# xxlong0/NeuralUDF

Hardware: NVIDIA H100
Metric: ray-samples/sec (render_core fwd+bwd) (higher is better)
Workload: dtype f32

## Files before the change

### neuraludf_b200/csrc/gemm_tc.cuh

```cuda
#pragma once
#include <cuda.h>
#include <cudaTypedefs.h>
#include <cuda_bf16.h>

#include "gemm_simt.cuh"

namespace nudf {
namespace tc {

constexpr int BM = 128;
constexpr int BN = 128;
constexpr int BK = 64;
constexpr int THREADS = 256;
constexpr int A_HALF_BYTES = BM * BK * 2;
constexpr int B_HALF_BYTES = BN * BK * 2;
__host__ __device__ constexpr int b_plane_bytes(int wn) { return wn * BK * 2; }
__host__ __device__ constexpr int acc_ld(int wn) { return wn + 4; }

__host__ __device__ inline int pad16(int n) { return (n + 15) & ~15; }
__host__ __device__ inline int pad64(int k) { return (k + 63) & ~63; }

__host__ __device__ inline uint32_t sw128(uint32_t row, uint32_t k) {
  return (row >> 3) * 1024u + (row & 7u) * 128u + ((((k >> 3) ^ (row & 7u)) & 7u) << 4) + ((k & 7u) << 1);
}

constexpr int TN_PS = 32;
constexpr int TN_RING = 4;
constexpr uint32_t TN_F32_OPND = TN_PS * BM * 4;
constexpr uint32_t TN_F32_STAGE = 2 * TN_F32_OPND;
constexpr uint32_t TN_PLANE = BM * TN_PS * 2;
constexpr uint32_t TN_PLANE_STAGE = 4 * TN_PLANE;
struct TnMaps { CUtensorMap a, b; };
__host__ __device__ inline uint32_t sw128_mn(uint32_t mn, uint32_t k) {
  return (mn >> 6) * 4096u + (k >> 3) * 1024u + (k & 7u) * 128u + ((((mn >> 3) ^ k) & 7u) << 4) + ((mn & 7u) << 1);
}

__device__ __forceinline__ uint32_t pack_bf16(float a, float b) {
  __nv_bfloat162 v = __floats2bfloat162_rn(a, b);
  return *reinterpret_cast<uint32_t*>(&v);
}
template <int NP>
__device__ __forceinline__ void split4(const float x[4], uint2 planes[NP]) {
  float r[4] = {x[0], x[1], x[2], x[3]};
#pragma unroll
  for (int p = 0; p < NP; ++p) {
    float h[4];
#pragma unroll
    for (int j = 0; j < 4; ++j) {
      h[j] = __bfloat162float(__float2bfloat16_rn(r[j]));
      r[j] -= h[j];
    }
    planes[p] = make_uint2(pack_bf16(h[0], h[1]), pack_bf16(h[2], h[3]));
  }
}
__host__ __device__ inline int nt_of(int np) { return np == 2 ? 256 : 128; }
__host__ __device__ inline int n_tiles(int N, int np) { return (N + nt_of(np) - 1) / nt_of(np); }
__host__ __device__ inline int tile_rows(int N, int t, int np) { int r = N - nt_of(np) * t; return pad16(r < nt_of(np) ? r : nt_of(np)); }
__host__ __device__ inline int64_t tile_elems(int N, int K, int t, int np) { return (int64_t)(pad64(K) / 64) * np * tile_rows(N, t, np) * 64; }
__host__ __device__ inline int64_t tile_offset(int N, int K, int t, int np) {
  int64_t o = 0;
  for (int i = 0; i < t; ++i) o += tile_elems(N, K, i, np);
  return o;
}
__host__ __device__ inline int64_t image_elems(int N, int K, int np) { return tile_offset(N, K, n_tiles(N, np), np); }

static __device__ __forceinline__ void tc_prep_weights_body(const float* __restrict__ W, int64_t ldw, int N, int K, int transposed, int np,
                                                            uint16_t* __restrict__ img, int64_t start, int64_t stride) {
  const int Kp = pad64(K);
  const int nt = n_tiles(N, np);
  int64_t total = 0;
  for (int t = 0; t < nt; ++t) total += (int64_t)tile_rows(N, t, np) * Kp;
  for (int64_t idx = start; idx < total; idx += stride) {
    int64_t rem = idx;
    int t = 0;
    while (rem >= (int64_t)tile_rows(N, t, np) * Kp) { rem -= (int64_t)tile_rows(N, t, np) * Kp; ++t; }
    const int rows = tile_rows(N, t, np);
    const int nl = (int)(rem / Kp), k = (int)(rem - (int64_t)nl * Kp);
    const int n = t * nt_of(np) + nl;
    float x = 0.f;
    if (n < N && k < K) x = transposed ? W[(int64_t)k * ldw + n] : W[(int64_t)n * ldw + k];
    const int s = k >> 6, kl = k & 63;
    uint16_t* base = img + tile_offset(N, K, t, np) + (int64_t)s * np * rows * 64;
    const uint32_t off = sw128((uint32_t)nl, (uint32_t)kl) >> 1;
    float r = x;
    for (int p = 0; p < np; ++p) {
      __nv_bfloat16 h = __float2bfloat16_rn(r);
      base[(int64_t)p * rows * 64 + off] = __bfloat16_as_ushort(h);
      r -= __bfloat162float(h);
    }
  }
}
static __global__ void tc_prep_weights_kernel(const float* __restrict__ W, int64_t ldw, int N, int K, int transposed, int np,
                                              uint16_t* __restrict__ img) {
  tc_prep_weights_body(W, ldw, N, K, transposed, np, img, (int64_t)blockIdx.x * blockDim.x + threadIdx.x, (int64_t)gridDim.x * blockDim.x);
}


__device__ __forceinline__ uint32_t smem_u32(const void* p) { return (uint32_t)__cvta_generic_to_shared(p); }
__device__ __forceinline__ uint8_t* align1024(uint8_t* p) {
  return reinterpret_cast<uint8_t*>((reinterpret_cast<uintptr_t>(p) + 1023) & ~(uintptr_t)1023);
}

__device__ __forceinline__ void mbar_init(uint64_t* bar, uint32_t count) {
  asm volatile("mbarrier.init.shared::cta.b64 [%0], %1;" ::"r"(smem_u32(bar)), "r"(count) : "memory");
}
__device__ __forceinline__ void mbar_arrive_expect_tx(uint64_t* bar, uint32_t bytes) {
  asm volatile("mbarrier.arrive.expect_tx.shared::cta.b64 _, [%0], %1;" ::"r"(smem_u32(bar)), "r"(bytes) : "memory");
}
__device__ __forceinline__ uint32_t mbar_try_wait(uint32_t addr, uint32_t parity) {
  uint32_t ok;
  asm volatile(
      "{\n"
      ".reg .pred p;\n"
      "mbarrier.try_wait.parity.shared::cta.b64 p, [%1], %2;\n"
      "selp.u32 %0, 1, 0, p;\n"
      "}\n"
      : "=r"(ok)
      : "r"(addr), "r"(parity)
// ... 74 lines not shown
        "=f"(d[37]), "=f"(d[38]), "=f"(d[39]), "=f"(d[40]), "=f"(d[41]), "=f"(d[42]), "=f"(d[43]), "=f"(d[44]), "=f"(d[45]),
        "=f"(d[46]), "=f"(d[47]), "=f"(d[48]), "=f"(d[49]), "=f"(d[50]), "=f"(d[51]), "=f"(d[52]), "=f"(d[53]), "=f"(d[54]),
        "=f"(d[55]), "=f"(d[56]), "=f"(d[57]), "=f"(d[58]), "=f"(d[59]), "=f"(d[60]), "=f"(d[61]), "=f"(d[62]), "=f"(d[63])
      : "l"(da), "l"(db), "r"(0u));
}

__device__ __forceinline__ void wgmma_256(float (&d)[128], uint64_t da, uint64_t db, uint32_t accumulate) {
  asm volatile(
      "{\n"
      ".reg .pred p;\n"
      "setp.ne.b32 p, %130, 0;\n"
      "wgmma.mma_async.sync.aligned.m64n256k16.f32.bf16.bf16 "
      "{%0, %1, %2, %3, %4, %5, %6, %7, %8, %9, %10, %11, %12, %13, %14, %15, %16, %17, %18, %19, %20, %21, %22, %23, %24, "
      "%25, %26, %27, %28, %29, %30, %31, %32, %33, %34, %35, %36, %37, %38, %39, %40, %41, %42, %43, %44, %45, %46, %47, "
      "%48, %49, %50, %51, %52, %53, %54, %55, %56, %57, %58, %59, %60, %61, %62, %63, %64, %65, %66, %67, %68, %69, %70, "
      "%71, %72, %73, %74, %75, %76, %77, %78, %79, %80, %81, %82, %83, %84, %85, %86, %87, %88, %89, %90, %91, %92, %93, "
      "%94, %95, %96, %97, %98, %99, %100, %101, %102, %103, %104, %105, %106, %107, %108, %109, %110, %111, %112, %113, "
      "%114, %115, %116, %117, %118, %119, %120, %121, %122, %123, %124, %125, %126, %127}, %128, %129, p, 1, 1, 0, 0;\n"
      "}\n"
      : "+f"(d[0]), "+f"(d[1]), "+f"(d[2]), "+f"(d[3]), "+f"(d[4]), "+f"(d[5]), "+f"(d[6]), "+f"(d[7]), "+f"(d[8]),
        "+f"(d[9]), "+f"(d[10]), "+f"(d[11]), "+f"(d[12]), "+f"(d[13]), "+f"(d[14]), "+f"(d[15]), "+f"(d[16]), "+f"(d[17]),
        "+f"(d[18]), "+f"(d[19]), "+f"(d[20]), "+f"(d[21]), "+f"(d[22]), "+f"(d[23]), "+f"(d[24]), "+f"(d[25]), "+f"(d[26]),
        "+f"(d[27]), "+f"(d[28]), "+f"(d[29]), "+f"(d[30]), "+f"(d[31]), "+f"(d[32]), "+f"(d[33]), "+f"(d[34]), "+f"(d[35]),
        "+f"(d[36]), "+f"(d[37]), "+f"(d[38]), "+f"(d[39]), "+f"(d[40]), "+f"(d[41]), "+f"(d[42]), "+f"(d[43]), "+f"(d[44]),
        "+f"(d[45]), "+f"(d[46]), "+f"(d[47]), "+f"(d[48]), "+f"(d[49]), "+f"(d[50]), "+f"(d[51]), "+f"(d[52]), "+f"(d[53]),
        "+f"(d[54]), "+f"(d[55]), "+f"(d[56]), "+f"(d[57]), "+f"(d[58]), "+f"(d[59]), "+f"(d[60]), "+f"(d[61]), "+f"(d[62]),
        "+f"(d[63]), "+f"(d[64]), "+f"(d[65]), "+f"(d[66]), "+f"(d[67]), "+f"(d[68]), "+f"(d[69]), "+f"(d[70]), "+f"(d[71]),
        "+f"(d[72]), "+f"(d[73]), "+f"(d[74]), "+f"(d[75]), "+f"(d[76]), "+f"(d[77]), "+f"(d[78]), "+f"(d[79]), "+f"(d[80]),
        "+f"(d[81]), "+f"(d[82]), "+f"(d[83]), "+f"(d[84]), "+f"(d[85]), "+f"(d[86]), "+f"(d[87]), "+f"(d[88]), "+f"(d[89]),
        "+f"(d[90]), "+f"(d[91]), "+f"(d[92]), "+f"(d[93]), "+f"(d[94]), "+f"(d[95]), "+f"(d[96]), "+f"(d[97]), "+f"(d[98]),
        "+f"(d[99]), "+f"(d[100]), "+f"(d[101]), "+f"(d[102]), "+f"(d[103]), "+f"(d[104]), "+f"(d[105]), "+f"(d[106]),
        "+f"(d[107]), "+f"(d[108]), "+f"(d[109]), "+f"(d[110]), "+f"(d[111]), "+f"(d[112]), "+f"(d[113]), "+f"(d[114]),
        "+f"(d[115]), "+f"(d[116]), "+f"(d[117]), "+f"(d[118]), "+f"(d[119]), "+f"(d[120]), "+f"(d[121]), "+f"(d[122]),
        "+f"(d[123]), "+f"(d[124]), "+f"(d[125]), "+f"(d[126]), "+f"(d[127])
      : "l"(da), "l"(db), "r"(accumulate));
}

template <int WN>
__device__ __forceinline__ void wgmma_n(float (&d)[WN / 2], uint64_t da, uint64_t db, uint32_t accumulate) {
  if constexpr (WN == 256) wgmma_256(d, da, db, accumulate);
  else wgmma_128(d, da, db, accumulate);
}
template <int NP, int WN>
__device__ __forceinline__ void mma_slice(float (&d)[WN / 2], uint32_t a, uint32_t a_stride, uint32_t b, uint32_t b_stride, bool zero_first) {
  auto desc = [](uint32_t base, uint32_t stride, int p, int j) { return make_desc(base + p * stride + 32u * j); };
#pragma unroll
  for (int j = 0; j < BK / 16; ++j) {
    const uint32_t acc0 = (zero_first && j == 0) ? 0u : 1u;
    if constexpr (NP == 2) {
      wgmma_n<WN>(d, desc(a, a_stride, 1, j), desc(b, b_stride, 0, j), acc0);
      wgmma_n<WN>(d, desc(a, a_stride, 0, j), desc(b, b_stride, 1, j), 1u);
      wgmma_n<WN>(d, desc(a, a_stride, 0, j), desc(b, b_stride, 0, j), 1u);
    } else {
      wgmma_n<WN>(d, desc(a, a_stride, 2, j), desc(b, b_stride, 0, j), acc0);
      wgmma_n<WN>(d, desc(a, a_stride, 0, j), desc(b, b_stride, 2, j), 1u);
      wgmma_n<WN>(d, desc(a, a_stride, 1, j), desc(b, b_stride, 1, j), 1u);
      wgmma_n<WN>(d, desc(a, a_stride, 1, j), desc(b, b_stride, 0, j), 1u);
      wgmma_n<WN>(d, desc(a, a_stride, 0, j), desc(b, b_stride, 1, j), 1u);
    }
  }
}
__device__ __forceinline__ void mma_slice_mn(float (&d)[64], uint32_t a, uint32_t b, bool zero_first) {
#pragma unroll
  for (int j = 0; j < TN_PS / 16; ++j) {
    const uint32_t acc0 = (zero_first && j == 0) ? 0u : 1u;
    const uint32_t aj = a + 2048u * j, bj = b + 2048u * j;
    wgmma_128<1>(d, make_desc_mn(aj + TN_PLANE), make_desc_mn(bj), acc0);
    wgmma_128<1>(d, make_desc_mn(aj), make_desc_mn(bj + TN_PLANE), 1u);
    wgmma_128<1>(d, make_desc_mn(aj), make_desc_mn(bj), 1u);
  }
}

template <int WN>
__device__ __forceinline__ void acc_to_smem(const float (&d)[WN / 2], float* acc_s, int wg, int wtid) {
  constexpr int LD = acc_ld(WN);
  const int r = 64 * wg + 16 * (wtid >> 5) + ((wtid & 31) >> 2);
  const int c = 2 * (wtid & 3);
#pragma unroll
  for (int g = 0; g < WN / 8; ++g) {
    *reinterpret_cast<float2*>(acc_s + r * LD + 8 * g + c) = make_float2(d[4 * g], d[4 * g + 1]);
    *reinterpret_cast<float2*>(acc_s + (r + 8) * LD + 8 * g + c) = make_float2(d[4 * g + 2], d[4 * g + 3]);
  }
}
template <int WN, class Epi>
__device__ __forceinline__ void tile_epilogue(const float* acc_s, int64_t m0, int64_t M, int n0, int n_valid_end, const Epi& epi, int tid) {
  constexpr int LD = acc_ld(WN);
  const int cq = tid & 31;
#pragma unroll 1
  for (int h = 0; h < WN / 128; ++h) {
    const int cl = 128 * h + 4 * cq;
    const int col = n0 + cl;
    int nv = n_valid_end - col;
    nv = nv < 4 ? nv : 4;
    if (nv <= 0) break;
    for (int r0 = tid >> 5; r0 < BM; r0 += 2 * (THREADS / 32)) {
      typename Epi::Aux aux[2];
#pragma unroll
      for (int i = 0; i < 2; ++i) {
        const int64_t row = m0 + r0 + i * (THREADS / 32);
        if (row < M) epi.load(row, col, nv, aux[i]);
      }
#pragma unroll
      for (int i = 0; i < 2; ++i) {
        const int r = r0 + i * (THREADS / 32);
        const int64_t row = m0 + r;
        if (row < M) {
          const float4 t = *reinterpret_cast<const float4*>(acc_s + r * LD + cl);
          const float x[4] = {t.x, t.y, t.z, t.w};
          epi.apply(row, col, x, nv, aux[i]);
        }
      }
    }
  }
}

template <int NT>
__device__ __forceinline__ void fetch_a(const float* __restrict__ A, int64_t lda, int64_t m0, int64_t M, int k0, int K, int tid,
                                        bool vec_ok, float4 (&v)[BM * 16 / NT]) {
  const int c = tid & 15;
  const int rsub = tid >> 4;
  const int k = k0 + c * 4;
#pragma unroll
  for (int pass = 0; pass < BM * 16 / NT; ++pass) {
    const int64_t row = m0 + pass * (NT / 16) + rsub;
    v[pass] = make_float4(0.f, 0.f, 0.f, 0.f);
    if (row < M) {
      const float* p = A + row * lda + k;
      if (vec_ok && k + 3 < K) {
        v[pass] = *reinterpret_cast<const float4*>(p);
      } else {
        if (k + 0 < K) v[pass].x = p[0];
        if (k + 1 < K) v[pass].y = p[1];
        if (k + 2 < K) v[pass].z = p[2];
        if (k + 3 < K) v[pass].w = p[3];
      }
    }
  }
}
template <int NP, int NT>
__device__ __forceinline__ void store_a(const float4 (&v)[BM * 16 / NT], uint8_t* sa, int tid) {
  const int c = tid & 15;
  const int rsub = tid >> 4;
#pragma unroll
  for (int pass = 0; pass < BM * 16 / NT; ++pass) {
    const float x[4] = {v[pass].x, v[pass].y, v[pass].z, v[pass].w};
    uint2 pl[NP];
    split4<NP>(x, pl);
    const uint32_t off = sw128((uint32_t)(pass * (NT / 16) + rsub), (uint32_t)(c * 4));
#pragma unroll
    for (int p = 0; p < NP; ++p) *reinterpret_cast<uint2*>(sa + p * A_HALF_BYTES + off) = pl[p];
  }
}
template <int NP, int NT>
__device__ __forceinline__ void stage_a_direct(const float* __restrict__ A, int64_t lda, int64_t m0, int64_t M, int k0, int K,
                                               uint8_t* sa, int tid, bool vec_ok) {
  float4 v[BM * 16 / NT];
  fetch_a<NT>(A, lda, m0, M, k0, K, tid, vec_ok, v);
  store_a<NP, NT>(v, sa, tid);
}

__device__ __forceinline__ void fetch_block_t(const float* __restrict__ X, int64_t ld, int m0, int m_total, int r0, int rows,
                                              int64_t k0, int64_t k_end, int lane, bool vec_ok, float4 (&v)[8][2]) {
  const int mq = lane & 7, kq = lane >> 3;
  if (r0 + 4 * mq >= rows) return;
  const int m = m0 + r0 + 4 * mq;
#pragma unroll
  for (int q = 0; q < 8; ++q) {
#pragma unroll
    for (int kk = 0; kk < 2; ++kk) {
      const int64_t k = k0 + 2 * (4 * q + kq) + kk;
      v[q][kk] = make_float4(0.f, 0.f, 0.f, 0.f);
      if (k < k_end) {
        const float* p = X + k * ld + m;
        if (vec_ok && m + 3 < m_total) {
          v[q][kk] = *reinterpret_cast<const float4*>(p);
        } else {
          if (m + 0 < m_total) v[q][kk].x = p[0];
          if (m + 1 < m_total) v[q][kk].y = p[1];
          if (m + 2 < m_total) v[q][kk].z = p[2];
          if (m + 3 < m_total) v[q][kk].w = p[3];
        }
      }
    }
  }
}
template <bool CSUM = false>
__device__ __forceinline__ void store_block_t(const float4 (&v)[8][2], int r0, int rows, uint8_t* s_hi, uint8_t* s_lo, int lane,
                                              float* csum = nullptr) {
  const int mq = lane & 7, kq = lane >> 3;
  if (r0 + 4 * mq >= rows) return;
  if (CSUM) {
#pragma unroll
    for (int q = 0; q < 8; ++q) {
      csum[0] += v[q][0].x + v[q][1].x; csum[1] += v[q][0].y + v[q][1].y;
      csum[2] += v[q][0].z + v[q][1].z; csum[3] += v[q][0].w + v[q][1].w;
    }
  }
#pragma unroll
  for (int q = 0; q < 8; ++q) {
    const float x0[4] = {v[q][0].x, v[q][0].y, v[q][0].z, v[q][0].w};
    const float x1[4] = {v[q][1].x, v[q][1].y, v[q][1].z, v[q][1].w};
#pragma unroll
    for (int j = 0; j < 4; ++j) {
      const float h0 = __bfloat162float(__float2bfloat16_rn(x0[j])), h1 = __bfloat162float(__float2bfloat16_rn(x1[j]));
      const uint32_t off = sw128((uint32_t)(r0 + 4 * mq + j), (uint32_t)(2 * (4 * q + kq)));
      *reinterpret_cast<uint32_t*>(s_hi + off) = pack_bf16(h0, h1);
      *reinterpret_cast<uint32_t*>(s_lo + off) = pack_bf16(x0[j] - h0, x1[j] - h1);
    }
  }
}

template <int NP, int WN, class Epi>
__global__ void __launch_bounds__(THREADS, 1)
gemm_w_kernel(const float* __restrict__ A, int64_t lda, int64_t M, int N, int K, const uint16_t* __restrict__ img, Epi epi) {
  static_assert(WN == 128 || (WN == 256 && NP == 2), "WN = 256 only with 2 planes (3 planes need 2 x WN/2 accumulators)");
  extern __shared__ uint8_t smem_raw[];
  uint8_t* smem = align1024(smem_raw);
  const int tid = threadIdx.x, wg = tid >> 7;
  const int n_ct = (N + WN - 1) / WN;
  const int n0 = (int)(blockIdx.x % (unsigned)n_ct) * WN;
  const int64_t m0 = (int64_t)(blockIdx.x / (unsigned)n_ct) * BM;
  const int t = n0 / nt_of(NP);
  const int rows_t = tile_rows(N, t, NP);
  const int row_in_tile = n0 - t * nt_of(NP);
  int rows_h = rows_t - row_in_tile; rows_h = rows_h < WN ? rows_h : WN;
  const int n_slices = pad64(K) / 64;
  constexpr uint32_t B_PLANE = b_plane_bytes(WN);
  const uint32_t a_bytes = NP * A_HALF_BYTES, stage_bytes = a_bytes + NP * B_PLANE;
  uint64_t* full = reinterpret_cast<uint64_t*>(smem + 2 * stage_bytes);
  const uint16_t* img_t = img + tile_offset(N, K, t, NP) + (int64_t)row_in_tile * 64;
  const bool vec_ok = ((lda & 3) == 0) && aligned16(A);

  auto issue_copies = [&](int ks) {
    uint8_t* st = smem + (ks & 1) * stage_bytes;
    const uint32_t wb = (uint32_t)rows_h * 128u;
    mbar_arrive_expect_tx(&full[ks & 1], NP * wb);
    for (int p = 0; p < NP; ++p) bulk_g2s(st + a_bytes + p * B_PLANE, img_t + ((int64_t)ks * NP + p) * rows_t * 64, wb, &full[ks & 1]);
  };
  if (tid == 0) {
    mbar_init(&full[0], 1);
    mbar_init(&full[1], 1);
    fence_barrier_init();
  }
  __syncthreads();
  if (n_slices > 0) {
    if (tid == 0) issue_copies(0);
    stage_a_direct<NP, THREADS>(A, lda, m0, M, 0, K, smem, tid, vec_ok);
    fence_proxy_async();
  }
  __syncthreads();
  constexpr int NACC = WN / 2, NTOT = NP == 3 ? 64 : 1;
  float acc[NACC], tot[NTOT], acc2[NTOT];
#pragma unroll
  for (int q = 0; q < NACC; ++q) acc[q] = 0.f;
#pragma unroll
  for (int q = 0; q < NTOT; ++q) tot[q] = 0.f;
  for (int ks = 0; ks < n_slices; ++ks) {
    const int s = ks & 1;
    if (tid == 0 && ks + 1 < n_slices) issue_copies(ks + 1);
    mbar_wait(&full[s], (uint32_t)((ks >> 1) & 1));
    const uint32_t st = smem_u32(smem + s * stage_bytes);
    wg_fence();
    mma_slice<NP, WN>(acc, st + wg * (64 * 128), A_HALF_BYTES, st + a_bytes, B_PLANE, NP == 3 || ks == 0);
    wg_commit();
    if (ks + 1 < n_slices) stage_a_direct<NP, THREADS>(A, lda, m0, M, (ks + 1) * BK, K, smem + (s ^ 1) * stage_bytes, tid, vec_ok);
    wg_wait_all();
    if constexpr (NP == 3) {
      static_assert(BK / 16 == 4, "four hi * hi steps per K slice");
      auto hi_hi = [&](float (&d)[64], int j) {
        wg_fence();
        wgmma_128_fresh(d, make_desc(st + wg * (64 * 128) + 32u * j), make_desc(st + a_bytes + 32u * j));
        wg_commit();
      };
      auto add_unbiased = [&](float (&d)[64]) {
        fence_operand(d);
#pragma unroll
        for (int q = 0; q < 64; ++q) tot[q] += unbias_rz(d[q]);
      };
      hi_hi(acc2, 0);
      fence_operand(acc);
#pragma unroll
      for (int q = 0; q < 64; ++q) tot[q] += acc[q];
      hi_hi(acc, 1);
      wg_wait_but_one();
      add_unbiased(acc2);
      hi_hi(acc2, 2);
      wg_wait_but_one();
      add_unbiased(acc);
      hi_hi(acc, 3);
      wg_wait_but_one();
      add_unbiased(acc2);
      wg_wait_all();
      add_unbiased(acc);
    }
    fence_proxy_async();
    __syncthreads();
  }
  float* acc_s = reinterpret_cast<float*>(smem);
  if constexpr (NP == 3) acc_to_smem<WN>(tot, acc_s, wg, tid & 127);
  else acc_to_smem<WN>(acc, acc_s, wg, tid & 127);
  __syncthreads();
  tile_epilogue<WN>(acc_s, m0, M, n0, N, epi, tid);
}

template <class Epi, bool RING>
__global__ void __launch_bounds__(THREADS, 1)
gemm_tn_kernel(const float* __restrict__ A, int64_t lda, const float* __restrict__ B, int64_t ldb, int M, int N, int64_t K, int64_t k_chunk,
               Epi epi, float* __restrict__ colsum, float* __restrict__ cs_ws, const __grid_constant__ TnMaps maps) {
  extern __shared__ uint8_t smem_raw[];
  uint8_t* smem = align1024(smem_raw);
  const int tid = threadIdx.x, wg = tid >> 7, warp = tid >> 5, lane = tid & 31;
  const int m0 = blockIdx.x * BM;
  const int n0 = blockIdx.y * BN;
  const int64_t kb = (int64_t)blockIdx.z * k_chunk;
  const int64_t ke = (kb + k_chunk < K) ? kb + k_chunk : K;
  const bool do_csum = colsum != nullptr && blockIdx.y == 0;
  float csum[4] = {0.f, 0.f, 0.f, 0.f};
  if (ke <= kb) return;
  float acc[64];
#pragma unroll
  for (int q = 0; q < 64; ++q) acc[q] = 0.f;
  if constexpr (RING) {
    uint8_t* ring = smem;
    uint8_t* planes = smem + TN_RING * TN_F32_STAGE;
    float* cs_part = reinterpret_cast<float*>(planes + 2 * TN_PLANE_STAGE);
    uint64_t* full = reinterpret_cast<uint64_t*>(cs_part + 4 * BM);
    const int n_sl = (int)((ke - kb + TN_PS - 1) / TN_PS);
    const int opnd = warp >> 2, kq = warp & 3;

    auto issue = [&](int i) {
      const int r = i % TN_RING;
      const int k0 = (int)(kb + (int64_t)i * TN_PS);
      uint8_t* st = ring + r * TN_F32_STAGE;
      mbar_arrive_expect_tx(&full[r], TN_F32_STAGE);
      tma_load_2d(st, &maps.a, m0, k0, &full[r]);
      tma_load_2d(st + TN_F32_OPND, &maps.b, n0, k0, &full[r]);
    };
    auto split = [&](int i, uint8_t* dst) {
      const int r = i % TN_RING;
      mbar_wait(&full[r], (uint32_t)((i / TN_RING) & 1));
      const float* f = reinterpret_cast<const float*>(ring + r * TN_F32_STAGE + opnd * TN_F32_OPND) + 4 * lane;
      uint8_t* hi = dst + opnd * 2 * TN_PLANE;
      const int64_t k0 = kb + (int64_t)i * TN_PS;
#pragma unroll
      for (int q = 0; q < TN_PS / 8; ++q) {
        float4 v[2];
#pragma unroll
        for (int kk = 0; kk < 2; ++kk) {
          const int p = 8 * q + 2 * kq + kk;
          v[kk] = k0 + p < ke ? *reinterpret_cast<const float4*>(f + p * BM) : make_float4(0.f, 0.f, 0.f, 0.f);
        }
        if (opnd == 0 && do_csum) {
          csum[0] += v[0].x + v[1].x; csum[1] += v[0].y + v[1].y;
          csum[2] += v[0].z + v[1].z; csum[3] += v[0].w + v[1].w;
        }
#pragma unroll
        for (int kk = 0; kk < 2; ++kk) {
          const float x[4] = {v[kk].x, v[kk].y, v[kk].z, v[kk].w};
          uint2 pl[2];
          split4<2>(x, pl);
          const uint32_t off = sw128_mn(4u * lane, (uint32_t)(8 * q + 2 * kq + kk));
          *reinterpret_cast<uint2*>(hi + off) = pl[0];
          *reinterpret_cast<uint2*>(hi + TN_PLANE + off) = pl[1];
        }
      }
    };
    if (tid == 0) {
      for (int r = 0; r < TN_RING; ++r) mbar_init(&full[r], 1);
      fence_barrier_init();
      for (int i = 0; i < TN_RING && i < n_sl; ++i) issue(i);
    }
    __syncthreads();
    split(0, planes);
    fence_proxy_async();
    __syncthreads();
    if (tid == 0 && TN_RING < n_sl) issue(TN_RING);
    for (int i = 0; i < n_sl; ++i) {
      const int s = i & 1;
      const uint32_t st = smem_u32(planes + s * TN_PLANE_STAGE);
// ... 10 lines not shown
#pragma unroll
      for (int j = 0; j < 4; ++j) cs_part[kq * BM + 4 * lane + j] = csum[j];
  } else {
    int rows_b = N - n0; rows_b = pad16(rows_b < BN ? rows_b : BN);
    const int n_sl = (int)((ke - kb + BK - 1) / BK);
    constexpr uint32_t stage_bytes = 2u * A_HALF_BYTES + 2u * B_HALF_BYTES;
    const bool a_vec = ((lda & 3) == 0) && aligned16(A) && ((m0 & 3) == 0);
    const bool b_vec = ((ldb & 3) == 0) && aligned16(B);
    const bool b_warp = warp >= 4 && 32 * (warp - 4) < rows_b;
    float4 v[8][2];

    auto fetch = [&](int i) {
      const int64_t k0 = kb + (int64_t)i * BK;
      if (warp < 4) fetch_block_t(A, lda, m0, M, 32 * warp, BM, k0, ke, lane, a_vec, v);
      else if (b_warp) fetch_block_t(B, ldb, n0, N, 32 * (warp - 4), rows_b, k0, ke, lane, b_vec, v);
    };
    auto store = [&](uint8_t* st) {
      if (warp < 4) {
        if (do_csum) store_block_t<true>(v, 32 * warp, BM, st, st + A_HALF_BYTES, lane, csum);
        else store_block_t(v, 32 * warp, BM, st, st + A_HALF_BYTES, lane);
      } else if (b_warp) {
        store_block_t(v, 32 * (warp - 4), rows_b, st + 2 * A_HALF_BYTES, st + 2 * A_HALF_BYTES + B_HALF_BYTES, lane);
      }
    };
    fetch(0);
    store(smem);
    if (n_sl > 1) fetch(1);
    fence_proxy_async();
    __syncthreads();
    for (int i = 0; i < n_sl; ++i) {
      const int s = i & 1;
      const uint32_t st = smem_u32(smem + s * stage_bytes);
      wg_fence();
      mma_slice<2, BN>(acc, st + wg * (64 * 128), A_HALF_BYTES, st + 2 * A_HALF_BYTES, B_HALF_BYTES, i == 0);
      wg_commit();
      if (i + 1 < n_sl) {
        store(smem + (s ^ 1) * stage_bytes);
        if (i + 2 < n_sl) fetch(i + 2);
      }
      wg_wait_all();
      fence_proxy_async();
      __syncthreads();
    }
    if (do_csum && warp < 4) {
#pragma unroll
      for (int j = 0; j < 4; ++j) {
        csum[j] += __shfl_xor_sync(0xffffffffu, csum[j], 8);
        csum[j] += __shfl_xor_sync(0xffffffffu, csum[j], 16);
      }
      const int m = m0 + 32 * warp + 4 * (lane & 7);
      if ((lane >> 3) == 0)
#pragma unroll
        for (int j = 0; j < 4; ++j)
          if (m + j < M) {
            if (cs_ws != nullptr) cs_ws[(int64_t)blockIdx.z * M + m + j] = csum[j];
            else colsum[m + j] += csum[j];
          }
    }
  }
  float* acc_s = reinterpret_cast<float*>(smem);
  acc_to_smem<BN>(acc, acc_s, wg, tid & 127);
  __syncthreads();
  if constexpr (RING) {
    const float* cs_part = reinterpret_cast<const float*>(smem + TN_RING * TN_F32_STAGE + 2 * TN_PLANE_STAGE);
    if (do_csum && tid < BM && m0 + tid < M) {
      const float c = (cs_part[tid] + cs_part[BM + tid]) + (cs_part[2 * BM + tid] + cs_part[3 * BM + tid]);
      if (cs_ws != nullptr) cs_ws[(int64_t)blockIdx.z * M + m0 + tid] = c;
      else colsum[m0 + tid] += c;
    }
  }
  tile_epilogue<BN>(acc_s, m0, M, n0, N, epi, tid);
}

static inline int sm_count() {
  static int n = 0;
  if (n == 0) {
    int dev = 0;
    if (cudaGetDevice(&dev) != cudaSuccess || cudaDeviceGetAttribute(&n, cudaDevAttrMultiProcessorCount, dev) != cudaSuccess || n <= 0) n = 132;
  }
  return n;
}


constexpr size_t w_smem_bytes(int np, int wn) { return 2 * (size_t)np * (A_HALF_BYTES + b_plane_bytes(wn)) + 2 * sizeof(uint64_t) + 1024; }
static_assert(BM * acc_ld(2 * BN) * sizeof(float) <= 2 * 2 * (size_t)(A_HALF_BYTES + b_plane_bytes(2 * BN)), "accumulator tile");
constexpr size_t TN_SMEM = 2 * (size_t)(2 * A_HALF_BYTES + 2 * B_HALF_BYTES) + 2 * sizeof(uint64_t) + 1024;
constexpr size_t TN_RING_SMEM = (size_t)TN_RING * TN_F32_STAGE + 2 * TN_PLANE_STAGE + 4 * BM * sizeof(float) + TN_RING * sizeof(uint64_t) + 1024;
static_assert(BM * acc_ld(BN) * sizeof(float) <= (size_t)TN_RING * TN_F32_STAGE, "accumulator tile in the ring");
static_assert(TN_RING_SMEM <= 227 * 1024, "one CTA per SM");

template <int NP, int WN, class Epi>
static inline int gemm_w_launch(const float* A, int64_t lda, int64_t M, int N, int K, const uint16_t* img, const Epi& epi, cudaStream_t st) {
  constexpr size_t smem = w_smem_bytes(NP, WN);
  static bool attr_set = false;
  if (!attr_set) {
    NUDF_CUDA_OK(cudaFuncSetAttribute(gemm_w_kernel<NP, WN, Epi>, cudaFuncAttributeMaxDynamicSharedMemorySize, (int)smem));
    attr_set = true;
  }
  const unsigned grid = (unsigned)(cdiv(M, BM) * cdiv(N, WN));
  LaunchTimer lt_(epi_family<Epi>::value, st);
  gemm_w_kernel<NP, WN, Epi><<<grid, THREADS, smem, st>>>(A, lda, M, N, K, img, epi);
  NUDF_LAUNCH_OK();
  return 0;
}
template <int NP, class Epi>
static inline int gemm_w(const float* A, int64_t lda, int64_t M, int N, int K, const uint16_t* img, const Epi& epi, cudaStream_t st) {
  if (M <= 0 || N <= 0) return 0;
  if constexpr (NP == 2)
    if (N > BN) return gemm_w_launch<2, 2 * BN, Epi>(A, lda, M, N, K, img, epi, st);
  return gemm_w_launch<NP, BN, Epi>(A, lda, M, N, K, img, epi, st);
}

constexpr int TN_WAVE_CTAS = 132;
constexpr int64_t TN_MIN_POINTS = 512;
static inline int64_t tn_k_chunk(int M, int N, int64_t K) {
  const int64_t tiles = cdiv(M, BM) * cdiv(N, BN);
  int64_t splits = TN_WAVE_CTAS / tiles;
  if (splits > cdiv(K, TN_MIN_POINTS)) splits = cdiv(K, TN_MIN_POINTS);
  splits = ws_splits(splits < 1 ? 1 : (int)splits, (int64_t)M * N + M);
  return round_up(cdiv(K, splits), BK);
}

static inline int tn_tensor_map(CUtensorMap* map, const float* X, int64_t ld, int cols, int64_t rows) {
  static PFN_cuTensorMapEncodeTiled encode = nullptr;
  if (encode == nullptr) {
    void* fn = nullptr;
    cudaDriverEntryPointQueryResult q;
    if (cudaGetDriverEntryPoint("cuTensorMapEncodeTiled", &fn, cudaEnableDefault, &q) != cudaSuccess || q != cudaDriverEntryPointSuccess ||
        fn == nullptr) {
      nudf::set_error("cuTensorMapEncodeTiled is not available from the driver");
      return -2;
    }
    encode = reinterpret_cast<PFN_cuTensorMapEncodeTiled>(fn);
  }
  const cuuint64_t dims[2] = {(cuuint64_t)cols, (cuuint64_t)rows};
  const cuuint64_t strides[1] = {(cuuint64_t)ld * sizeof(float)};
  const cuuint32_t box[2] = {(cuuint32_t)BM, (cuuint32_t)TN_PS};
  const cuuint32_t elem[2] = {1, 1};
  const CUresult r = encode(map, CU_TENSOR_MAP_DATA_TYPE_FLOAT32, 2, const_cast<float*>(X), dims, strides, box, elem,
                            CU_TENSOR_MAP_INTERLEAVE_NONE, CU_TENSOR_MAP_SWIZZLE_NONE, CU_TENSOR_MAP_L2_PROMOTION_L2_256B,
                            CU_TENSOR_MAP_FLOAT_OOB_FILL_NONE);
  if (r != CUDA_SUCCESS) {
    nudf::set_error("cuTensorMapEncodeTiled failed (%d)", (int)r);
    return -2;
  }
  return 0;
}
template <class Epi, bool RING>
static inline int gemm_tn_launch(dim3 grid, const float* A, int64_t lda, const float* B, int64_t ldb, int M, int N, int64_t K,
                                 int64_t k_chunk, const Epi& epi, float* colsum, float* cs_ws, cudaStream_t st) {
  constexpr size_t smem = RING ? TN_RING_SMEM : TN_SMEM;
  static bool attr_set = false;
  if (!attr_set) {
    NUDF_CUDA_OK(cudaFuncSetAttribute(gemm_tn_kernel<Epi, RING>, cudaFuncAttributeMaxDynamicSharedMemorySize, (int)smem));
    attr_set = true;
  }
  TnMaps maps{};
  if constexpr (RING) {
    if (int rc = tn_tensor_map(&maps.a, A, lda, M, K)) return rc;
    if (int rc = tn_tensor_map(&maps.b, B, ldb, N, K)) return rc;
  }
  gemm_tn_kernel<Epi, RING><<<grid, THREADS, smem, st>>>(A, lda, B, ldb, M, N, K, k_chunk, epi, colsum, cs_ws, maps);
  NUDF_LAUNCH_OK();
  return 0;
}
template <class Epi>
static inline int gemm_tn(const float* A, int64_t lda, const float* B, int64_t ldb, int M, int N, int64_t K, const Epi& epi,
                          cudaStream_t st, float* colsum_a = nullptr) {
  if (M <= 0 || N <= 0 || K <= 0) return 0;
  const int64_t k_chunk = tn_k_chunk(M, N, K);
  const int splits = (int)cdiv(K, k_chunk);
  dim3 grid((unsigned)cdiv(M, BM), (unsigned)cdiv(N, BN), (unsigned)splits);
  LaunchTimer lt_(FAM_TC_WGRAD, st);
  const bool ring = (lda & 3) == 0 && (ldb & 3) == 0 && aligned16(A) && aligned16(B);
  if (splits == 1) {
    if (ring) return gemm_tn_launch<Epi, true>(grid, A, lda, B, ldb, M, N, K, k_chunk, epi, colsum_a, nullptr, st);
    return gemm_tn_launch<Epi, false>(grid, A, lda, B, ldb, M, N, K, k_chunk, epi, colsum_a, nullptr, st);
  }
  float* ws = split_workspace(st);
  if (ws == nullptr) return -2;
  float* cs = ws + (int64_t)splits * M * N;
  const EpiSplitStore e{ws, (int64_t)M * N, N};
  if (int rc = ring ? gemm_tn_launch<EpiSplitStore, true>(grid, A, lda, B, ldb, M, N, K, k_chunk, e, colsum_a, cs, st)
                    : gemm_tn_launch<EpiSplitStore, false>(grid, A, lda, B, ldb, M, N, K, k_chunk, e, colsum_a, cs, st))
    return rc;
  if (int rc = splitk_reduce(ws, splits, M, N, epi, st)) return rc;
  return colsum_a != nullptr ? vec_reduce(cs, splits, M, colsum_a, st) : 0;
}

struct PrepWJob { const float* W; uint16_t* img; int ldw, N, K, transposed, np; };
struct PrepWJobs { int n; PrepWJob j[64]; };
static __global__ void tc_prep_weights_jobs_kernel(const __grid_constant__ PrepWJobs jobs) {
  const PrepWJob& J = jobs.j[blockIdx.y];
  tc_prep_weights_body(J.W, J.ldw, J.N, J.K, J.transposed, J.np, J.img, (int64_t)blockIdx.x * blockDim.x + threadIdx.x,
                       (int64_t)gridDim.x * blockDim.x);
}
static inline int prep_weights_jobs(const PrepWJobs& jobs, cudaStream_t st) {
  if (jobs.n <= 0) return 0;
  int64_t mx = 0;
  for (int i = 0; i < jobs.n; ++i) {
    int64_t total = 0;
    for (int t = 0; t < n_tiles(jobs.j[i].N, jobs.j[i].np); ++t) total += (int64_t)tile_rows(jobs.j[i].N, t, jobs.j[i].np) * pad64(jobs.j[i].K);
    mx = total > mx ? total : mx;
  }
  int blocks = (int)((mx + 255) / 256);
  if (blocks > 1024) blocks = 1024;
  tc_prep_weights_jobs_kernel<<<dim3((unsigned)blocks, (unsigned)jobs.n), 256, 0, st>>>(jobs);
  NUDF_LAUNCH_OK();
  return 0;
}

static inline int prep_weights(const float* W, int64_t ldw, int N, int K, int transposed, int np, uint16_t* img, cudaStream_t st) {
  int64_t total = 0;
  for (int t = 0; t < n_tiles(N, np); ++t) total += (int64_t)tile_rows(N, t, np) * pad64(K);
  int blocks = (int)((total + 255) / 256);
  if (blocks > 4096) blocks = 4096;
  tc_prep_weights_kernel<<<blocks, 256, 0, st>>>(W, ldw, N, K, transposed, np, img);
  NUDF_LAUNCH_OK();
  return 0;
}

}
}
```

Measured before the change: 7.146 million.

## Stream fp32 activations via TMA ring and split in place for two-plane GEMM

For the two-plane forward GEMM with aligned A, activations are now fetched as fp32 tiles by TMA into a 3-4 deep ring of slots. Each slot is converted in place into bf16 hi/lo planes, replacing the synchronous per-thread global loads in stage_a_direct. The goal is to hide global latency for the A operand behind the wgmma work. It adds extra __syncthreads per slice and uses more shared memory, and the epilogue now keeps more rows' aux loads in flight for non-default epilogue families.

Result: faster. 7.552 million, median of 6 (+5.7%).

```diff
diff --git a/neuraludf_b200/csrc/gemm_tc.cuh b/neuraludf_b200/csrc/gemm_tc.cuh
--- a/neuraludf_b200/csrc/gemm_tc.cuh
+++ b/neuraludf_b200/csrc/gemm_tc.cuh
@@ -34,6 +34,10 @@
 __host__ __device__ inline uint32_t sw128_mn(uint32_t mn, uint32_t k) {
   return (mn >> 6) * 4096u + (k >> 3) * 1024u + (k & 7u) * 128u + ((((mn >> 3) ^ k) & 7u) << 4) + ((mn & 7u) << 1);
 }
+
+constexpr uint32_t W_SLOT = BM * BK * 4;
+static_assert(W_SLOT == 2 * A_HALF_BYTES, "a slot holds exactly the two bf16 planes of its slice");
+__host__ __device__ constexpr int w_ring(int wn) { return wn == 256 ? 3 : 4; }
 
 __device__ __forceinline__ uint32_t pack_bf16(float a, float b) {
   __nv_bfloat162 v = __floats2bfloat162_rn(a, b);
@@ -274,9 +278,11 @@
     *reinterpret_cast<float2*>(acc_s + (r + 8) * LD + 8 * g + c) = make_float2(d[4 * g + 2], d[4 * g + 3]);
   }
 }
+template <class Epi> constexpr int epi_rows_in_flight() { return epi_family<Epi>::value == FAM_TC_OTHER ? 2 : 8; }
 template <int WN, class Epi>
 __device__ __forceinline__ void tile_epilogue(const float* acc_s, int64_t m0, int64_t M, int n0, int n_valid_end, const Epi& epi, int tid) {
   constexpr int LD = acc_ld(WN);
+  constexpr int EPI_ROWS = epi_rows_in_flight<Epi>();
   const int cq = tid & 31;
 #pragma unroll 1
   for (int h = 0; h < WN / 128; ++h) {
@@ -285,15 +291,15 @@
     int nv = n_valid_end - col;
     nv = nv < 4 ? nv : 4;
     if (nv <= 0) break;
-    for (int r0 = tid >> 5; r0 < BM; r0 += 2 * (THREADS / 32)) {
-      typename Epi::Aux aux[2];
-#pragma unroll
-      for (int i = 0; i < 2; ++i) {
+    for (int r0 = tid >> 5; r0 < BM; r0 += EPI_ROWS * (THREADS / 32)) {
+      typename Epi::Aux aux[EPI_ROWS];
+#pragma unroll
+      for (int i = 0; i < EPI_ROWS; ++i) {
         const int64_t row = m0 + r0 + i * (THREADS / 32);
         if (row < M) epi.load(row, col, nv, aux[i]);
       }
 #pragma unroll
-      for (int i = 0; i < 2; ++i) {
+      for (int i = 0; i < EPI_ROWS; ++i) {
         const int r = r0 + i * (THREADS / 32);
         const int64_t row = m0 + r;
         if (row < M) {
@@ -402,10 +408,12 @@
   }
 }
 
-template <int NP, int WN, class Epi>
+template <int NP, int WN, class Epi, bool RING>
 __global__ void __launch_bounds__(THREADS, 1)
-gemm_w_kernel(const float* __restrict__ A, int64_t lda, int64_t M, int N, int K, const uint16_t* __restrict__ img, Epi epi) {
+gemm_w_kernel(const float* __restrict__ A, int64_t lda, int64_t M, int N, int K, const uint16_t* __restrict__ img, Epi epi,
+              const __grid_constant__ CUtensorMap amap) {
   static_assert(WN == 128 || (WN == 256 && NP == 2), "WN = 256 only with 2 planes (3 planes need 2 x WN/2 accumulators)");
+  static_assert(!RING || NP == 2, "the ring path splits a slot into 2 planes in place");
   extern __shared__ uint8_t smem_raw[];
   uint8_t* smem = align1024(smem_raw);
   const int tid = threadIdx.x, wg = tid >> 7;
@@ -418,75 +426,133 @@
   int rows_h = rows_t - row_in_tile; rows_h = rows_h < WN ? rows_h : WN;
   const int n_slices = pad64(K) / 64;
   constexpr uint32_t B_PLANE = b_plane_bytes(WN);
-  const uint32_t a_bytes = NP * A_HALF_BYTES, stage_bytes = a_bytes + NP * B_PLANE;
-  uint64_t* full = reinterpret_cast<uint64_t*>(smem + 2 * stage_bytes);
   const uint16_t* img_t = img + tile_offset(N, K, t, NP) + (int64_t)row_in_tile * 64;
-  const bool vec_ok = ((lda & 3) == 0) && aligned16(A);
-
-  auto issue_copies = [&](int ks) {
-    uint8_t* st = smem + (ks & 1) * stage_bytes;
-    const uint32_t wb = (uint32_t)rows_h * 128u;
-    mbar_arrive_expect_tx(&full[ks & 1], NP * wb);
-    for (int p = 0; p < NP; ++p) bulk_g2s(st + a_bytes + p * B_PLANE, img_t + ((int64_t)ks * NP + p) * rows_t * 64, wb, &full[ks & 1]);
-  };
-  if (tid == 0) {
-    mbar_init(&full[0], 1);
-    mbar_init(&full[1], 1);
-    fence_barrier_init();
-  }
-  __syncthreads();
-  if (n_slices > 0) {
-    if (tid == 0) issue_copies(0);
-    stage_a_direct<NP, THREADS>(A, lda, m0, M, 0, K, smem, tid, vec_ok);
-    fence_proxy_async();
-  }
-  __syncthreads();
   constexpr int NACC = WN / 2, NTOT = NP == 3 ? 64 : 1;
   float acc[NACC], tot[NTOT], acc2[NTOT];
 #pragma unroll
   for (int q = 0; q < NACC; ++q) acc[q] = 0.f;
 #pragma unroll
   for (int q = 0; q < NTOT; ++q) tot[q] = 0.f;
-  for (int ks = 0; ks < n_slices; ++ks) {
-    const int s = ks & 1;
-    if (tid == 0 && ks + 1 < n_slices) issue_copies(ks + 1);
-    mbar_wait(&full[s], (uint32_t)((ks >> 1) & 1));
-    const uint32_t st = smem_u32(smem + s * stage_bytes);
-    wg_fence();
-    mma_slice<NP, WN>(acc, st + wg * (64 * 128), A_HALF_BYTES, st + a_bytes, B_PLANE, NP == 3 || ks == 0);
-    wg_commit();
-    if (ks + 1 < n_slices) stage_a_direct<NP, THREADS>(A, lda, m0, M, (ks + 1) * BK, K, smem + (s ^ 1) * stage_bytes, tid, vec_ok);
-    wg_wait_all();
-    if constexpr (NP == 3) {
-      static_assert(BK / 16 == 4, "four hi * hi steps per K slice");
-      auto hi_hi = [&](float (&d)[64], int j) {
-        wg_fence();
-        wgmma_128_fresh(d, make_desc(st + wg * (64 * 128) + 32u * j), make_desc(st + a_bytes + 32u * j));
-        wg_commit();
-      };
-      auto add_unbiased = [&](float (&d)[64]) {
-        fence_operand(d);
-#pragma unroll
-        for (int q = 0; q < 64; ++q) tot[q] += unbias_rz(d[q]);
-      };
-      hi_hi(acc2, 0);
-      fence_operand(acc);
-#pragma unroll
-      for (int q = 0; q < 64; ++q) tot[q] += acc[q];
-      hi_hi(acc, 1);
-      wg_wait_but_one();
-      add_unbiased(acc2);
-      hi_hi(acc2, 2);
-      wg_wait_but_one();
-      add_unbiased(acc);
-      hi_hi(acc, 3);
-      wg_wait_but_one();
-      add_unbiased(acc2);
+
+  if constexpr (RING) {
+    constexpr int NR = w_ring(WN);
+    constexpr uint32_t W_STAGE = 2 * B_PLANE;
+    uint8_t* wst = smem + NR * W_SLOT;
+    uint64_t* afull = reinterpret_cast<uint64_t*>(wst + 2 * W_STAGE);
+    uint64_t* wfull = afull + NR;
+    auto issue_a = [&](int i) {
+      const int r = i % NR;
+      mbar_arrive_expect_tx(&afull[r], W_SLOT);
+      tma_load_2d(smem + r * W_SLOT, &amap, i * BK, (int)m0, &afull[r]);
+    };
+    auto issue_w = [&](int ks) {
+      uint8_t* st = wst + (ks & 1) * W_STAGE;
+      const uint32_t wb = (uint32_t)rows_h * 128u;
+      mbar_arrive_expect_tx(&wfull[ks & 1], 2 * wb);
+      for (int p = 0; p < 2; ++p) bulk_g2s(st + p * B_PLANE, img_t + ((int64_t)ks * 2 + p) * rows_t * 64, wb, &wfull[ks & 1]);
+    };
+    auto split = [&](int i) {
+      uint8_t* slot = smem + (i % NR) * W_SLOT;
+      mbar_wait(&afull[i % NR], (uint32_t)((i / NR) & 1));
+      float4 v[BM * 16 / THREADS];
+      const float4* f = reinterpret_cast<const float4*>(slot) + (tid >> 4) * (BK / 4) + (tid & 15);
+#pragma unroll
+      for (int pass = 0; pass < BM * 16 / THREADS; ++pass) v[pass] = f[pass * (THREADS / 16) * (BK / 4)];
+      __syncthreads();
+      store_a<2, THREADS>(v, slot, tid);
+    };
+    if (tid == 0) {
+      for (int r = 0; r < NR; ++r) mbar_init(&afull[r], 1);
+      mbar_init(&wfull[0], 1);
+      mbar_init(&wfull[1], 1);
+      fence_barrier_init();
+      if (n_slices > 0) issue_w(0);
+      for (int i = 0; i < NR && i < n_slices; ++i) issue_a(i);
+    }
+    __syncthreads();
+    if (n_slices > 0) {
+      split(0);
+      fence_proxy_async();
+    }
+    __syncthreads();
+    for (int ks = 0; ks < n_slices; ++ks) {
+      const int s = ks & 1;
+      if (tid == 0 && ks + 1 < n_slices) issue_w(ks + 1);
+      mbar_wait(&wfull[s], (uint32_t)((ks >> 1) & 1));
+      const uint32_t sa = smem_u32(smem + (ks % NR) * W_SLOT), sb = smem_u32(wst + s * W_STAGE);
+      wg_fence();
+      mma_slice<2, WN>(acc, sa + wg * (64 * 128), A_HALF_BYTES, sb, B_PLANE, ks == 0);
+      wg_commit();
+      if (ks + 1 < n_slices) split(ks + 1);
       wg_wait_all();
-      add_unbiased(acc);
-    }
-    fence_proxy_async();
+      fence_proxy_async();
+      __syncthreads();
+      if (tid == 0 && ks + NR < n_slices) issue_a(ks + NR);
+    }
+  } else {
+    const uint32_t a_bytes = NP * A_HALF_BYTES, stage_bytes = a_bytes + NP * B_PLANE;
+    uint64_t* full = reinterpret_cast<uint64_t*>(smem + 2 * stage_bytes);
+    const bool vec_ok = ((lda & 3) == 0) && aligned16(A);
+
+    auto issue_copies = [&](int ks) {
+      uint8_t* st = smem + (ks & 1) * stage_bytes;
+      const uint32_t wb = (uint32_t)rows_h * 128u;
+      mbar_arrive_expect_tx(&full[ks & 1], NP * wb);
+      for (int p = 0; p < NP; ++p) bulk_g2s(st + a_bytes + p * B_PLANE, img_t + ((int64_t)ks * NP + p) * rows_t * 64, wb, &full[ks & 1]);
+    };
+    if (tid == 0) {
+      mbar_init(&full[0], 1);
+      mbar_init(&full[1], 1);
+      fence_barrier_init();
+    }
     __syncthreads();
+    if (n_slices > 0) {
+      if (tid == 0) issue_copies(0);
+      stage_a_direct<NP, THREADS>(A, lda, m0, M, 0, K, smem, tid, vec_ok);
+      fence_proxy_async();
+    }
+    __syncthreads();
+    for (int ks = 0; ks < n_slices; ++ks) {
+      const int s = ks & 1;
+      if (tid == 0 && ks + 1 < n_slices) issue_copies(ks + 1);
+      mbar_wait(&full[s], (uint32_t)((ks >> 1) & 1));
+      const uint32_t st = smem_u32(smem + s * stage_bytes);
+      wg_fence();
+      mma_slice<NP, WN>(acc, st + wg * (64 * 128), A_HALF_BYTES, st + a_bytes, B_PLANE, NP == 3 || ks == 0);
+      wg_commit();
+      if (ks + 1 < n_slices) stage_a_direct<NP, THREADS>(A, lda, m0, M, (ks + 1) * BK, K, smem + (s ^ 1) * stage_bytes, tid, vec_ok);
+      wg_wait_all();
+      if constexpr (NP == 3) {
+        static_assert(BK / 16 == 4, "four hi * hi steps per K slice");
+        auto hi_hi = [&](float (&d)[64], int j) {
+          wg_fence();
+          wgmma_128_fresh(d, make_desc(st + wg * (64 * 128) + 32u * j), make_desc(st + a_bytes + 32u * j));
+          wg_commit();
+        };
+        auto add_unbiased = [&](float (&d)[64]) {
+          fence_operand(d);
+#pragma unroll
+          for (int q = 0; q < 64; ++q) tot[q] += unbias_rz(d[q]);
+        };
+        hi_hi(acc2, 0);
+        fence_operand(acc);
+#pragma unroll
+        for (int q = 0; q < 64; ++q) tot[q] += acc[q];
+        hi_hi(acc, 1);
+        wg_wait_but_one();
+        add_unbiased(acc2);
+        hi_hi(acc2, 2);
+        wg_wait_but_one();
+        add_unbiased(acc);
+        hi_hi(acc, 3);
+        wg_wait_but_one();
+        add_unbiased(acc2);
+        wg_wait_all();
+        add_unbiased(acc);
+      }
+      fence_proxy_async();
+      __syncthreads();
+    }
   }
   float* acc_s = reinterpret_cast<float*>(smem);
   if constexpr (NP == 3) acc_to_smem<WN>(tot, acc_s, wg, tid & 127);
@@ -663,33 +729,68 @@
 }
 
 
+static inline int tensor_map_2d(CUtensorMap* map, const float* X, int64_t ld, int64_t cols, int64_t rows, int box_cols, int box_rows) {
+  static PFN_cuTensorMapEncodeTiled encode = nullptr;
+  if (encode == nullptr) {
+    void* fn = nullptr;
+    cudaDriverEntryPointQueryResult q;
+    if (cudaGetDriverEntryPoint("cuTensorMapEncodeTiled", &fn, cudaEnableDefault, &q) != cudaSuccess || q != cudaDriverEntryPointSuccess ||
+        fn == nullptr) {
+      nudf::set_error("cuTensorMapEncodeTiled is not available from the driver");
+      return -2;
+    }
+    encode = reinterpret_cast<PFN_cuTensorMapEncodeTiled>(fn);
+  }
+  const cuuint64_t dims[2] = {(cuuint64_t)cols, (cuuint64_t)rows};
+  const cuuint64_t strides[1] = {(cuuint64_t)ld * sizeof(float)};
+  const cuuint32_t box[2] = {(cuuint32_t)box_cols, (cuuint32_t)box_rows};
+  const cuuint32_t elem[2] = {1, 1};
+  const CUresult r = encode(map, CU_TENSOR_MAP_DATA_TYPE_FLOAT32, 2, const_cast<float*>(X), dims, strides, box, elem,
+                            CU_TENSOR_MAP_INTERLEAVE_NONE, CU_TENSOR_MAP_SWIZZLE_NONE, CU_TENSOR_MAP_L2_PROMOTION_L2_256B,
+                            CU_TENSOR_MAP_FLOAT_OOB_FILL_NONE);
+  if (r != CUDA_SUCCESS) {
+    nudf::set_error("cuTensorMapEncodeTiled failed (%d)", (int)r);
+    return -2;
+  }
+  return 0;
+}
 constexpr size_t w_smem_bytes(int np, int wn) { return 2 * (size_t)np * (A_HALF_BYTES + b_plane_bytes(wn)) + 2 * sizeof(uint64_t) + 1024; }
 static_assert(BM * acc_ld(2 * BN) * sizeof(float) <= 2 * 2 * (size_t)(A_HALF_BYTES + b_plane_bytes(2 * BN)), "accumulator tile");
-constexpr size_t TN_SMEM = 2 * (size_t)(2 * A_HALF_BYTES + 2 * B_HALF_BYTES) + 2 * sizeof(uint64_t) + 1024;
-constexpr size_t TN_RING_SMEM = (size_t)TN_RING * TN_F32_STAGE + 2 * TN_PLANE_STAGE + 4 * BM * sizeof(float) + TN_RING * sizeof(uint64_t) + 1024;
-static_assert(BM * acc_ld(BN) * sizeof(float) <= (size_t)TN_RING * TN_F32_STAGE, "accumulator tile in the ring");
-static_assert(TN_RING_SMEM <= 227 * 1024, "one CTA per SM");
-
-template <int NP, int WN, class Epi>
+constexpr size_t w_ring_operand_bytes(int wn) { return (size_t)w_ring(wn) * W_SLOT + 2 * 2 * (size_t)b_plane_bytes(wn); }
+constexpr size_t w_ring_smem_bytes(int wn) { return w_ring_operand_bytes(wn) + (w_ring(wn) + 2) * sizeof(uint64_t) + 1024; }
+static_assert(w_ring_smem_bytes(BN) <= 227 * 1024 && w_ring_smem_bytes(2 * BN) <= 227 * 1024, "one CTA per SM");
+static_assert(BM * acc_ld(BN) * sizeof(float) <= w_ring_operand_bytes(BN), "accumulator tile in the ring path's stages");
+static_assert(BM * acc_ld(2 * BN) * sizeof(float) <= w_ring_operand_bytes(2 * BN), "accumulator tile in the ring path's stages");
+
+template <int NP, int WN, class Epi, bool RING>
 static inline int gemm_w_launch(const float* A, int64_t lda, int64_t M, int N, int K, const uint16_t* img, const Epi& epi, cudaStream_t st) {
-  constexpr size_t smem = w_smem_bytes(NP, WN);
+  constexpr size_t smem = RING ? w_ring_smem_bytes(WN) : w_smem_bytes(NP, WN);
   static bool attr_set = false;
   if (!attr_set) {
-    NUDF_CUDA_OK(cudaFuncSetAttribute(gemm_w_kernel<NP, WN, Epi>, cudaFuncAttributeMaxDynamicSharedMemorySize, (int)smem));
+    NUDF_CUDA_OK(cudaFuncSetAttribute(gemm_w_kernel<NP, WN, Epi, RING>, cudaFuncAttributeMaxDynamicSharedMemorySize, (int)smem));
     attr_set = true;
   }
+  CUtensorMap amap{};
+  if constexpr (RING)
+    if (int rc = tensor_map_2d(&amap, A, lda, K, M, BK, BM)) return rc;
   const unsigned grid = (unsigned)(cdiv(M, BM) * cdiv(N, WN));
   LaunchTimer lt_(epi_family<Epi>::value, st);
-  gemm_w_kernel<NP, WN, Epi><<<grid, THREADS, smem, st>>>(A, lda, M, N, K, img, epi);
+  gemm_w_kernel<NP, WN, Epi, RING><<<grid, THREADS, smem, st>>>(A, lda, M, N, K, img, epi, amap);
   NUDF_LAUNCH_OK();
   return 0;
+}
+template <int NP, int WN, class Epi>
+static inline int gemm_w_path(const float* A, int64_t lda, int64_t M, int N, int K, const uint16_t* img, const Epi& epi, cudaStream_t st) {
+  if constexpr (NP == 2)
+    if (K > 0 && (lda & 3) == 0 && aligned16(A)) return gemm_w_launch<2, WN, Epi, true>(A, lda, M, N, K, img, epi, st);
+  return gemm_w_launch<NP, WN, Epi, false>(A, lda, M, N, K, img, epi, st);
 }
 template <int NP, class Epi>
 static inline int gemm_w(const float* A, int64_t lda, int64_t M, int N, int K, const uint16_t* img, const Epi& epi, cudaStream_t st) {
   if (M <= 0 || N <= 0) return 0;
   if constexpr (NP == 2)
-    if (N > BN) return gemm_w_launch<2, 2 * BN, Epi>(A, lda, M, N, K, img, epi, st);
-  return gemm_w_launch<NP, BN, Epi>(A, lda, M, N, K, img, epi, st);
+    if (N > BN) return gemm_w_path<2, 2 * BN, Epi>(A, lda, M, N, K, img, epi, st);
+  return gemm_w_path<NP, BN, Epi>(A, lda, M, N, K, img, epi, st);
 }
 
 constexpr int TN_WAVE_CTAS = 132;
@@ -702,31 +803,11 @@
   return round_up(cdiv(K, splits), BK);
 }
 
-static inline int tn_tensor_map(CUtensorMap* map, const float* X, int64_t ld, int cols, int64_t rows) {
-  static PFN_cuTensorMapEncodeTiled encode = nullptr;
-  if (encode == nullptr) {
-    void* fn = nullptr;
-    cudaDriverEntryPointQueryResult q;
-    if (cudaGetDriverEntryPoint("cuTensorMapEncodeTiled", &fn, cudaEnableDefault, &q) != cudaSuccess || q != cudaDriverEntryPointSuccess ||
-        fn == nullptr) {
-      nudf::set_error("cuTensorMapEncodeTiled is not available from the driver");
-      return -2;
-    }
-    encode = reinterpret_cast<PFN_cuTensorMapEncodeTiled>(fn);
-  }
-  const cuuint64_t dims[2] = {(cuuint64_t)cols, (cuuint64_t)rows};
-  const cuuint64_t strides[1] = {(cuuint64_t)ld * sizeof(float)};
-  const cuuint32_t box[2] = {(cuuint32_t)BM, (cuuint32_t)TN_PS};
-  const cuuint32_t elem[2] = {1, 1};
-  const CUresult r = encode(map, CU_TENSOR_MAP_DATA_TYPE_FLOAT32, 2, const_cast<float*>(X), dims, strides, box, elem,
-                            CU_TENSOR_MAP_INTERLEAVE_NONE, CU_TENSOR_MAP_SWIZZLE_NONE, CU_TENSOR_MAP_L2_PROMOTION_L2_256B,
-                            CU_TENSOR_MAP_FLOAT_OOB_FILL_NONE);
-  if (r != CUDA_SUCCESS) {
-    nudf::set_error("cuTensorMapEncodeTiled failed (%d)", (int)r);
-    return -2;
-  }
-  return 0;
-}
+constexpr size_t TN_SMEM = 2 * (size_t)(2 * A_HALF_BYTES + 2 * B_HALF_BYTES) + 2 * sizeof(uint64_t) + 1024;
+constexpr size_t TN_RING_SMEM = (size_t)TN_RING * TN_F32_STAGE + 2 * TN_PLANE_STAGE + 4 * BM * sizeof(float) + TN_RING * sizeof(uint64_t) + 1024;
+static_assert(BM * acc_ld(BN) * sizeof(float) <= (size_t)TN_RING * TN_F32_STAGE, "accumulator tile in the ring");
+static_assert(TN_RING_SMEM <= 227 * 1024, "one CTA per SM");
+
 template <class Epi, bool RING>
 static inline int gemm_tn_launch(dim3 grid, const float* A, int64_t lda, const float* B, int64_t ldb, int M, int N, int64_t K,
                                  int64_t k_chunk, const Epi& epi, float* colsum, float* cs_ws, cudaStream_t st) {
@@ -738,8 +819,8 @@
   }
   TnMaps maps{};
   if constexpr (RING) {
-    if (int rc = tn_tensor_map(&maps.a, A, lda, M, K)) return rc;
-    if (int rc = tn_tensor_map(&maps.b, B, ldb, N, K)) return rc;
+    if (int rc = tensor_map_2d(&maps.a, A, lda, M, K, BM, TN_PS)) return rc;
+    if (int rc = tensor_map_2d(&maps.b, B, ldb, N, K, BN, TN_PS)) return rc;
   }
   gemm_tn_kernel<Epi, RING><<<grid, THREADS, smem, st>>>(A, lda, B, ldb, M, N, K, k_chunk, epi, colsum, cs_ws, maps);
   NUDF_LAUNCH_OK();
```
